# eps696/aphantasia

Measured on AMD Instinct MI355X. Metric: optimization steps/sec @1280x720 ViT-B/32 samples=200, higher is better.
Workload: dtype f16 (MFMA operands, fp32 accumulate; fp32 residual stream / LayerNorm / softmax statistics / synth / sampler / loss / Adam)

## Files before the change

aphantasia_amd/_ffi.py:

```python
import ctypes
import os
from ctypes import POINTER, c_char_p, c_float, c_int, c_size_t, c_void_p

import torch

HERE = os.path.dirname(os.path.abspath(__file__))
LIB_PATH = os.path.join(HERE, 'libaphantasia_hip.so')

APH_OUT_NCHW_RAW, APH_OUT_NCHW_NORM, APH_OUT_PATCH_F16, APH_GRAD_PATCH_F16, APH_OUT_PATCH_F16_HILO, APH_OUT_PATCH_F32 = 0, 1, 2, 3, 4, 5
APH_AUG_STRIDE = 16
SIM_TYPES = {'cossim': 0, 'cos': 0, None: 0, 'mix': 1, 'ang': 2, 'dot': 3}


class SampleGeom(ctypes.Structure):
    _fields_ = [(n, c_int) for n in ('H', 'W', 'Hp', 'Wp', 'py0', 'px0', 'S', 'size', 'patch')]


_PROTOTYPES = {
    'aph_version': (c_int, []),
    'aph_last_error': (c_char_p, []),
    'aph_synth_plan_create': (c_int, [c_int, c_int, c_int, POINTER(c_void_p)]),
    'aph_synth_plan_destroy': (c_int, [c_void_p]),
    'aph_synth_fft_fwd': (c_int, [c_void_p, c_void_p, c_void_p, c_void_p, c_float, POINTER(c_float), c_int, c_void_p, c_void_p, c_void_p]),
    'aph_synth_fft_bwd': (c_int, [c_void_p, c_void_p, c_float, c_void_p, c_void_p, c_void_p, c_float, POINTER(c_float), c_int, c_void_p, c_void_p]),
# ... 14 lines not shown
    'aph_idwt_level_bwd': (c_int, [c_void_p, c_int, c_int, c_int, c_void_p, c_void_p, c_int, c_float, c_void_p, c_int, c_int, c_void_p, c_void_p]),
    'aph_sample_ws_bytes': (c_size_t, [POINTER(SampleGeom), c_int]),
    'aph_sample_fwd': (c_int, [POINTER(SampleGeom), c_void_p, c_void_p, c_void_p, c_void_p, c_void_p, c_int, c_void_p]),
    'aph_sample_bwd': (c_int, [POINTER(SampleGeom), c_void_p, c_float, c_void_p, c_void_p, c_void_p, c_void_p, c_int, c_void_p]),
    'aph_triangle_blur': (c_int, [c_void_p, c_int, c_int, c_int, c_int, c_float, c_float, c_void_p, c_void_p]),
    'aph_resize_bicubic': (c_int, [c_void_p, c_int, c_int, c_int, c_void_p, c_int, c_int, c_void_p]),
    'aph_flip_w': (c_int, [c_void_p, c_void_p, c_int, c_int, c_int, c_void_p, c_void_p]),
    'aph_grid_warp': (c_int, [c_void_p, c_void_p, c_int, c_int, c_int, c_float, c_float, c_float, c_float, c_float, c_void_p, c_void_p, c_void_p]),
    'aph_attn_test': (c_int, [c_void_p, c_void_p, c_void_p, c_void_p, c_void_p, c_void_p, c_int, c_int, c_int, c_int, c_void_p]),
    'aph_attn_f32_test': (c_int, [c_void_p, c_void_p, c_void_p, c_void_p, c_void_p, c_void_p, c_int, c_int, c_int, c_int, c_void_p]),
    'aph_frame_affine': (c_int, [c_void_p, c_int, c_int, c_int, POINTER(c_float), c_void_p, c_void_p]),
    'aph_patchify_f16': (c_int, [c_void_p, c_int, c_int, c_int, c_void_p, c_void_p]),
    'aph_patchify_f16_hilo': (c_int, [c_void_p, c_int, c_int, c_int, c_void_p, c_void_p]),
    'aph_patchify_f32': (c_int, [c_void_p, c_int, c_int, c_int, c_void_p, c_void_p]),
    'aph_unpatchify_f32': (c_int, [c_void_p, c_int, c_int, c_int, c_float, c_void_p, c_void_p]),
    'aph_vit_create': (c_int, [c_int, c_int, c_int, c_int, c_int, c_int, c_int, POINTER(c_void_p)]),
    'aph_vit_destroy': (c_int, [c_void_p]),
    'aph_vit_workspace_bytes': (c_size_t, [c_void_p]),
    'aph_vit_set_weight': (c_int, [c_void_p, c_char_p, c_void_p, c_size_t]),
    'aph_vit_forward': (c_int, [c_void_p, c_void_p, c_int, c_void_p, c_void_p]),
    'aph_vit_forward_hilo': (c_int, [c_void_p, c_void_p, c_int, c_void_p, c_void_p]),
    'aph_vit_enable_hilo': (c_int, [c_void_p]),
    'aph_vit_enable_f32': (c_int, [c_void_p]),
    'aph_vit_forward_f32': (c_int, [c_void_p, c_void_p, c_int, c_void_p, c_void_p]),
    'aph_vit_backward_f32': (c_int, [c_void_p, c_void_p, c_int, c_void_p, c_float, c_void_p]),
    'aph_vit_backward': (c_int, [c_void_p, c_void_p, c_int, c_void_p, c_float, c_void_p]),
    'aph_vit_backward_h': (c_int, [c_void_p, c_void_p, c_int, c_void_p, c_float, c_void_p]),
    'aph_vit_profile': (c_int, [c_void_p, c_int]),
    'aph_vit_profile_read': (c_int, [c_void_p, c_void_p, c_void_p, c_void_p]),
    'aph_gemm_set_mfma32': (c_int, [c_int]),
    'aph_vit_set_fuse_ln': (c_int, [c_int]),
    'aph_crop_adjoint_set_gather': (c_int, [c_int]),
    'aph_crop_adjoint_set_shape': (c_int, [c_int, c_int, c_int, c_int, c_int]),
    'aph_vit_set_grad_stream_f16': (c_int, [c_int]),
    'aph_gemm_set_ws_min_tiles': (c_int, [c_int]),
    'aph_gemm_set_ws_pgroup': (c_int, [c_int]),
    'aph_gemm_set_rs': (c_int, [c_int]),
    'aph_mfma_rate': (c_int, [c_int, c_int, c_void_p, c_void_p, c_void_p]),
    'aph_gemm_rs_probe': (c_int, [c_void_p, c_void_p, c_int, c_int, c_int, c_void_p, c_int, c_void_p, c_void_p]),
    'aph_gemm_ws_probe': (c_int, [c_void_p, c_void_p, c_int, c_int, c_int, c_void_p, c_void_p, c_void_p, c_int, c_void_p, c_void_p]),
    'aph_gemm_f32_test': (c_int, [c_void_p, c_int, c_int, c_void_p, c_int, c_int, c_int, c_int, c_void_p, c_int, c_void_p, c_void_p, c_int, c_void_p, c_size_t, c_void_p]),
    'aph_gemm_f16': (c_int, [c_void_p, c_void_p, c_int, c_int, c_int, c_void_p, c_void_p]),
    'aph_gemm_f16_ld': (c_int, [c_void_p, c_int, c_void_p, c_int, c_int, c_int, c_int, c_void_p, c_int, c_void_p]),
    'aph_gemm_f16_epi_test': (c_int, [c_void_p, c_int, c_void_p, c_int, c_int, c_int, c_int, c_void_p, c_int, c_void_p, c_void_p, c_void_p, c_float, c_int,
                                      c_int, c_int, c_int, c_void_p, c_size_t, c_int, c_void_p]),
    'aph_ln_test': (c_int, [c_int, c_int, c_int, c_int, c_int, c_int, c_int, c_void_p, c_void_p, c_void_p, c_void_p, c_void_p, c_void_p, c_void_p,
                            c_void_p, c_void_p, c_void_p, c_void_p, c_void_p, c_void_p, c_void_p]),
    'aph_sim_loss': (c_int, [c_void_p, c_int, c_int, c_void_p, c_void_p, POINTER(c_float), c_int, c_int, c_int, c_int, c_int, c_float, c_float, c_void_p, c_void_p, c_void_p, c_void_p]),
    'aph_axpy_f32': (c_int, [c_void_p, c_void_p, c_float, c_size_t, c_void_p]),
    'aph_rgb_to_u8': (c_int, [c_void_p, c_int, c_int, c_float, c_void_p, c_void_p]),
    'aph_linear_head': (c_int, [c_void_p, c_int, c_int, c_void_p, c_float, c_float, c_float, c_float, c_void_p, c_void_p, c_void_p]),
    'aph_comm_unique_id': (c_int, [c_void_p]),
    'aph_comm_init': (c_int, [c_int, c_int, c_void_p, POINTER(c_void_p)]),
    'aph_allreduce_f32': (c_int, [c_void_p, c_void_p, c_size_t, c_void_p]),
    'aph_comm_ranks': (c_int, [c_void_p, POINTER(c_int)]),
    'aph_comm_destroy': (c_int, [c_void_p]),
    'aph_adam_step': (c_int, [c_void_p, c_void_p, c_void_p, c_void_p, c_void_p, c_void_p, c_int, c_size_t, c_void_p]),
    'aph_adam_step_guarded': (c_int, [c_void_p, c_void_p, c_void_p, c_void_p, c_void_p, c_void_p, c_int, c_size_t, c_void_p, c_void_p]),
}

EXPORTS = tuple(_PROTOTYPES)

class Library:

    def __init__(self, path):
        if not os.path.isfile(path):
# ... 45 lines not shown
```

aphantasia_amd/csrc/sampler.hip:

```cpp
#include <cstring>
#include <cstdlib>
#include <type_traits>

#include "sampler_layout.h"
#include "sampler_crop.h"
#include "sampler_crop_adjoint.h"
#include "sampler_warp.h"

namespace aph {

struct Nchw { int s, c, i, j; };
__device__ __forceinline__ Nchw nchw_of(size_t idx, int R) {
  return Nchw{(int)(idx / ((size_t)3 * R * R)), (int)((idx / ((size_t)R * R)) % 3), (int)((idx / R) % R), (int)(idx % R)};
}

__global__ void patchify_kernel(const float* __restrict__ x, half_t* __restrict__ out, int S, int R, int p, int hilo) {
  const size_t n = (size_t)S * 3 * R * R;
  const Layout<APH_OUT_PATCH_F16> L(R, p);
  for (size_t idx = (size_t)blockIdx.x * blockDim.x + threadIdx.x; idx < n; idx += (size_t)gridDim.x * blockDim.x) {
    const Nchw e = nchw_of(idx, R);
    const size_t o = L.index(e.s, e.c, e.i, e.j);
    const half_t h = (half_t)x[idx];
    if (!hilo) { out[o] = h; continue; }
    const size_t q = L.hilo_index(o);
// ... 20 lines not shown

using namespace aph;

static Geom to_geom(const aph_sample_geom* g) { return Geom{g->H, g->W, g->Hp, g->Wp, g->py0, g->px0, g->S, g->size, g->patch}; }

static int check_geom(const aph_sample_geom* g, int out_mode, const char* who, int max_mode = 2) {
  if (!g) return aph_fail(APH_ERR_ARG, "%s: null geometry", who);
  if (out_mode == APH_OUT_PATCH_F16_HILO && max_mode == 2) max_mode = APH_OUT_PATCH_F16_HILO;
  if (out_mode == APH_OUT_PATCH_F32) max_mode = APH_OUT_PATCH_F32;
  if (g->S < 1 || g->size < 1 || g->H < 1 || g->W < 1 || g->Hp < g->H || g->Wp < g->W)
    return aph_fail(APH_ERR_ARG, "%s: bad geometry S=%d size=%d H=%d W=%d Hp=%d Wp=%d", who, g->S, g->size, g->H, g->W, g->Hp, g->Wp);
  if (out_mode < 0 || out_mode > max_mode || (out_mode == APH_GRAD_PATCH_F16 && max_mode != APH_GRAD_PATCH_F16))
    return aph_fail(APH_ERR_ARG, "%s: bad out_mode %d", who, out_mode);
  if (out_mode >= APH_OUT_PATCH_F16 && (g->patch < 1 || g->size % g->patch || (g->patch & (g->patch - 1))))
    return aph_fail(APH_ERR_ARG, "%s: size %d not divisible by patch %d, or patch not a power of two", who, g->size, g->patch);
  return APH_OK;
}

namespace {
template <int... MODES> struct Modes {};
template <int... MODES, class F>
bool dispatch_out(Modes<MODES...>, int out_mode, F&& f) {
  return ((out_mode == MODES ? (f(std::integral_constant<int, MODES>{}), true) : false) || ...);
}
using FwdModes = Modes<APH_OUT_NCHW_RAW, APH_OUT_NCHW_NORM, APH_OUT_PATCH_F16, APH_OUT_PATCH_F32, APH_OUT_PATCH_F16_HILO>;
using GradModes = Modes<APH_OUT_NCHW_RAW, APH_OUT_NCHW_NORM, APH_OUT_PATCH_F16, APH_GRAD_PATCH_F16>;

size_t tab_bytes(const Geom& g) {
  const size_t maxcs = (size_t)(g.Hp < g.Wp ? g.Hp : g.Wp);
  return ((size_t)g.S * 2 * maxcs * sizeof(AdjEntry) + 255) & ~(size_t)255;
}
size_t scratch_floats(const Geom& g) { return (size_t)g.S * 4 * g.size * g.size; }
size_t strip_bytes(const Geom& g) { return ((size_t)(8 * (size_t)strip_cap(g) + 8) * sizeof(int) + 255) & ~(size_t)255; }
int* ws_strips(void* ws, const Geom& g) { return reinterpret_cast<int*>(static_cast<char*>(ws) + tab_bytes(g)); }
float* ws_scratch(void* ws, const Geom& g) { return reinterpret_cast<float*>(static_cast<char*>(ws) + tab_bytes(g) + strip_bytes(g)); }
}

extern "C" {

int aph_crop_adjoint_set_shape(int rb, int cpt, int nbc, int nseg, int order) {
  CropAdjointShape& v = crop_adjoint_shape();
  v.rb = rb; v.cpt = cpt; v.nbc = nbc; v.nseg = nseg; v.order = order;
  return APH_OK;
}
int aph_crop_adjoint_set_gather(int on) {
  const int prev = crop_adjoint_gather();
  crop_adjoint_gather() = on ? 1 : 0;
  return prev;
}

size_t aph_sample_ws_bytes(const aph_sample_geom* gg, int with_aug) {
  if (!gg || gg->S < 1 || gg->size < 1 || gg->Hp < 1 || gg->Wp < 1) return 0;
  const Geom g = to_geom(gg);
  return tab_bytes(g) + strip_bytes(g) + (with_aug ? 2 * scratch_floats(g) * sizeof(float) : 0);
}

int aph_sample_fwd(const aph_sample_geom* gg, const float* rgb, const int32_t* table_, const float* aug, void* ws,
                   void* out, int out_mode, void* stream_) {
  APH_TRY
  if (int e = check_geom(gg, out_mode, "aph_sample_fwd")) return e;
  if (!rgb || !table_ || !out || !ws) return aph_fail(APH_ERR_ARG, "aph_sample_fwd: null argument (the workspace of aph_sample_ws_bytes is required)");
  hipStream_t st = (hipStream_t)stream_;
  const Geom g = to_geom(gg);
  const int n = g.size;
  const int* table = (const int*)table_;
  int* strips = ws_strips(ws, g);
  if (!aug) {
    if (!dispatch_out(FwdModes{}, out_mode, [&](auto m) { launch_crop_resize<decltype(m)::value>(rgb, table, out, g, strips, st); })) return aph_fail(APH_ERR_ARG, "aph_sample_fwd: no kernel for out_mode %d", out_mode);
    return aph_check_launch("aph_sample_fwd");
  }
  float* A = ws_scratch(ws, g);
  float* Bv = A + scratch_floats(g);
  const dim3 grid((n + 31) / 32, (n + 7) / 8, g.S), block(256);
  launch_crop_resize<APH_SCRATCH_HWC4>(rgb, table, (void*)A, g, strips, st);
  APH_LAUNCH(persp_kernel, grid, block, 0, st, (const float*)A, aug, Bv, n);
  if (!dispatch_out(FwdModes{}, out_mode, [&](auto m) { APH_LAUNCH(rotate_emit_kernel<decltype(m)::value>, grid, block, 0, st, (const float*)A, (const float*)Bv, aug, out, n, g.patch); })) return aph_fail(APH_ERR_ARG, "aph_sample_fwd: no kernel for out_mode %d", out_mode);
  return aph_check_launch("aph_sample_fwd");
  APH_CATCH
}

int aph_sample_bwd(const aph_sample_geom* gg, const void* gout, float gscale, const int32_t* table_, const float* aug,
                   void* ws, float* grgb, int out_mode, void* stream_) {
  APH_TRY
  if (int e = check_geom(gg, out_mode, "aph_sample_bwd", APH_GRAD_PATCH_F16)) return e;
  if (out_mode == APH_OUT_PATCH_F32) out_mode = APH_OUT_PATCH_F16;
  if (!gout || !table_ || !grgb || !ws) return aph_fail(APH_ERR_ARG, "aph_sample_bwd: null argument (the workspace of aph_sample_ws_bytes is required)");
  hipStream_t st = (hipStream_t)stream_;
  const Geom g = to_geom(gg);
  const int n = g.size;
  const int* table = (const int*)table_;
  AdjEntry* tab = static_cast<AdjEntry*>(ws);
  int rc = APH_OK;
  if (!aug) {
    if (!dispatch_out(GradModes{}, out_mode, [&](auto m) { rc = launch_crop_adjoint<decltype(m)::value>(gout, gscale, table, grgb, g, tab, st); })) return aph_fail(APH_ERR_ARG, "aph_sample_bwd: no kernel for out_mode %d", out_mode);
    return rc ? rc : aph_check_launch("aph_sample_bwd");
  }
  float* dA = ws_scratch(ws, g);
  float* dB = dA + scratch_floats(g);
  const dim3 grid((n + 31) / 32, (n + 7) / 8, g.S), block(256);
  if (!dispatch_out(GradModes{}, out_mode, [&](auto m) { APH_LAUNCH(rotate_emit_adjoint_kernel<decltype(m)::value>, grid, block, 0, st, gout, aug, dA, dB, n, g.patch); })) return aph_fail(APH_ERR_ARG, "aph_sample_bwd: no kernel for out_mode %d", out_mode);
  APH_LAUNCH(persp_adjoint_kernel, grid, block, 0, st, (const float*)dB, aug, dA, n);
  rc = launch_crop_adjoint<APH_OUT_NCHW_RAW>((const void*)dA, gscale, table, grgb, g, tab, st);
  return rc ? rc : aph_check_launch("aph_sample_bwd");
  APH_CATCH
}

int aph_patchify_f16(const float* x, int S, int R, int patch, void* out, void* stream_) {
  APH_TRY
  if (!x || !out || S < 1 || R < 1 || patch < 1 || R % patch) return aph_fail(APH_ERR_ARG, "aph_patchify_f16: bad argument");
// ... 41 lines not shown
```

aphantasia_amd/csrc/sampler_crop.h:

```cpp
#pragma once
#include "sampler_layout.h"

namespace aph {

__device__ __forceinline__ void bicubic3(const float* __restrict__ rgb, const Geom& g, const CutBox& b, int i, int j, float v[3]) {
  const float sy = b.scale * (float)i, sx = b.scale * (float)j;
  const int y0 = (int)floorf(sy), x0 = (int)floorf(sx);
  float wy[4], wx[4];
  cubic_w(sy - (float)y0, wy);
  cubic_w(sx - (float)x0, wx);
  int ry[4], rx[4];
#pragma unroll
  for (int k = 0; k < 4; ++k) {
    int yy = y0 - 1 + k; yy = yy < 0 ? 0 : (yy > b.cs - 1 ? b.cs - 1 : yy);
    int xx = x0 - 1 + k; xx = xx < 0 ? 0 : (xx > b.cs - 1 ? b.cs - 1 : xx);
    ry[k] = wrap(b.oy + yy - g.py0, g.H);
    rx[k] = wrap(b.ox + xx - g.px0, g.W);
  }
  if (wave_all(rx[3] == rx[0] + 3)) {
    F4u t[3][4];
#pragma unroll
    for (int c = 0; c < 3; ++c)
#pragma unroll
      for (int a = 0; a < 4; ++a) t[c][a] = *reinterpret_cast<const F4u*>(rgb + ((size_t)c * g.H + ry[a]) * g.W + rx[0]);
#pragma unroll
    for (int c = 0; c < 3; ++c) {
      float acc = 0.f;
#pragma unroll
      for (int a = 0; a < 4; ++a) acc += (t[c][a].v[0] * wx[0] + t[c][a].v[1] * wx[1] + t[c][a].v[2] * wx[2] + t[c][a].v[3] * wx[3]) * wy[a];
      v[c] = acc;
    }
    return;
  }
#pragma unroll
// ... 2 lines not shown
    float acc = 0.f;
#pragma unroll
    for (int a = 0; a < 4; ++a) {
      const float* row = pl + (size_t)ry[a] * g.W;
      acc += (row[rx[0]] * wx[0] + row[rx[1]] * wx[1] + row[rx[2]] * wx[2] + row[rx[3]] * wx[3]) * wy[a];
    }
    v[c] = acc;
  }
}

constexpr int kStripPx = 16;
constexpr int kUnitRows = 4;
constexpr int kStripSlots = 768;

__global__ __launch_bounds__(1024) void strip_list_kernel(const int* __restrict__ table, int* __restrict__ lists, int* __restrict__ counts, int cap, Geom g, int strip_px) {
  __shared__ int cnt[8];
  if (threadIdx.x < 8) cnt[threadIdx.x] = 0;
  __syncthreads();
  const int groups = (g.size + kUnitRows - 1) / kUnitRows, units = g.S * groups;
  for (int u = threadIdx.x; u < units; u += blockDim.x) {
    const int s = u / groups, rg = u - s * groups;
    const CutBox b = load_cut(table, s, g.size);
    int i = rg * kUnitRows + kUnitRows / 2; i = i > g.size - 1 ? g.size - 1 : i;
    int yy = (int)floorf(b.scale * (float)i); yy = yy > b.cs - 1 ? b.cs - 1 : yy;
    const int yc = wrap(b.oy + yy - g.py0, g.H);
    const int xcd = (yc / strip_px) & 7;
    const int pos = atomicAdd(&cnt[xcd], 1);
    lists[xcd * cap + pos] = u;
  }
  __syncthreads();
  if (threadIdx.x < 8) counts[threadIdx.x] = cnt[threadIdx.x];
}

template <int OUT>
__global__ __launch_bounds__(256) void crop_resize_strips_kernel(const float* __restrict__ rgb, const int* __restrict__ table, void* __restrict__ out, Geom g,
                                                                 const int* __restrict__ lists, const int* __restrict__ counts, int cap) {
  const int xcd = blockIdx.x & 7, slot = blockIdx.x >> 3, nslot = gridDim.x >> 3;
  const int count = counts[xcd], groups = (g.size + kUnitRows - 1) / kUnitRows, n = g.size;
  for (int it = slot; it < count; it += nslot) {
    const int u = lists[xcd * cap + it];
    const int s = u / groups, rg = u - s * groups;
    const CutBox b = load_cut(table, s, n);
    for (int p = threadIdx.x; p < kUnitRows * n; p += blockDim.x) {
      const int di = p / n, j = p - di * n, i = rg * kUnitRows + di;
      if (i >= n) continue;
      float v[3];
      bicubic3(rgb, g, b, i, j, v);
      emit3<OUT>(out, s, i, j, n, g.patch, v[0], v[1], v[2]);
    }
  }
}

inline int strip_cap(const Geom& g) { return g.S * ((g.size + kUnitRows - 1) / kUnitRows); }

template <int OUT>
void launch_crop_resize(const float* rgb, const int* table, void* out, const Geom& g, int* lists, hipStream_t st) {
  int* counts = lists + 8 * (size_t)strip_cap(g);
  APH_LAUNCH(strip_list_kernel, dim3(1), dim3(1024), 0, st, table, lists, counts, strip_cap(g), g, kStripPx);
  APH_LAUNCH(crop_resize_strips_kernel<OUT>, dim3(8 * kStripSlots), dim3(256), 0, st, rgb, table, out, g, (const int*)lists, (const int*)counts, strip_cap(g));
}

}
```

aphantasia_amd/csrc/sampler_crop_adjoint.h:

```cpp
#pragma once
#include <type_traits>
#include "sampler_layout.h"

namespace aph {

struct AdjEntry { int off[4]; float w[4]; };

__device__ __forceinline__ float tap_weight(float scale, int i, int cs, int q) {
  const float sy = scale * (float)i;
  const int y0 = (int)floorf(sy);
  float wv[4];
  cubic_w(sy - (float)y0, wv);
  float w = 0.f;
#pragma unroll
  for (int k = 0; k < 4; ++k) {
    int yy = y0 - 1 + k; yy = yy < 0 ? 0 : (yy > cs - 1 ? cs - 1 : yy);
    if (yy == q) w += wv[k];
  }
  return w;
}

template <class Hit, class Put>
__device__ __forceinline__ void wave0_compact(int n, int* count, Hit hit, Put put) {
  int c = 0;
  for (int k0 = 0; k0 < n; k0 += 64) {
    const int k = k0 + (int)threadIdx.x;
    const bool h = k < n && hit(k);
    const unsigned long long m = __ballot(h);
    if (h) put(c + __popcll(m & ((1ull << threadIdx.x) - 1ull)), k);
    c += __popcll(m);
  }
  if (threadIdx.x == 0) *count = c;
}

template <int OUT, int NC>
__device__ __forceinline__ void upsample_cut_sum(const void* __restrict__ gout, size_t gb, const Layout<OUT>& L, float scale, int cs, int yc, int xc, float (&acc)[NC]) {
  for (int i = 0; i < L.size; ++i) {
    const float wy = tap_weight(scale, i, cs, yc);
    if (wy == 0.f) continue;
    for (int j = 0; j < L.size; ++j) {
      const float wx = tap_weight(scale, j, cs, xc);
      if (wx == 0.f) continue;
      const int o = L.rowpart(i) + L.colpart(j);
#pragma unroll
      for (int ch = 0; ch < NC; ++ch) acc[ch] += wy * wx * L.load(gout, gb + o + ch * L.chan_stride());
    }
  }
}

template <int OUT>
__global__ void tap_table_kernel(const int* __restrict__ table, AdjEntry* __restrict__ tab, int maxcs, Geom g) {
  const int s = blockIdx.z, isrow = blockIdx.y == 0;
  const int q = blockIdx.x * blockDim.x + threadIdx.x;
  const int cs = table[3 * s];
  if (q >= cs || q >= maxcs) return;
  const Layout<OUT> L(g.size, g.patch);
  AdjEntry e;
#pragma unroll
  for (int a = 0; a < 4; ++a) { e.off[a] = 0; e.w[a] = 0.f; }
  const float scale = cut_scale(cs, g.size);
  if (scale >= 1.0f) {
    const float inv = 1.0f / scale;
    int lo = (int)floorf((float)(q - 2) * inv) - 1, hi = (int)floorf((float)(q + 2) * inv) + 1;
    lo = lo < 0 ? 0 : lo; hi = hi > g.size - 1 ? g.size - 1 : hi;
    int n = 0;
    for (int i = lo; i <= hi && n < 4; ++i) {
      const float w = tap_weight(scale, i, cs, q);
      if (w != 0.f || n > 0) {
        e.w[n] = w;
        e.off[n] = isrow ? L.rowpart(i) : L.colpart(i);
        ++n;
      }
    }
  }
  tab[((size_t)s * 2 + (isrow ? 0 : 1)) * maxcs + q] = e;
}

template <int OUT>
__global__ __launch_bounds__(256) void crop_resize_adjoint_kernel(const void* __restrict__ gout, float gscale,
                                                                  const int* __restrict__ table, float* __restrict__ grgb, Geom g,
                                                                  const AdjEntry* __restrict__ tab, int maxcs) {
  constexpr int MAXV = 1024, NB = 8;
  __shared__ int vlist[MAXV];
  __shared__ int vcount;
  __shared__ AdjEntry ent[NB][32];
  __shared__ int vinfo[NB][3];
  const int tx = threadIdx.x & 15, ty = threadIdx.x >> 4;
  const int ntx_ = (g.W + 15) / 16, nty_ = (g.H + 15) / 16;
  const int xcd_ = blockIdx.x & 7, idx_ = blockIdx.x >> 3;
  const int lrow_ = idx_ / ntx_, bx_ = idx_ - lrow_ * ntx_, by_ = lrow_ * 8 + xcd_;
  if (by_ >= nty_) return;
  const int x = bx_ * 16 + tx, y = by_ * 16 + ty;
  const bool live = x < g.W && y < g.H;
  const int nay = (g.Hp + g.H - 1) / g.H, nax = (g.Wp + g.W - 1) / g.W;
  const int nvirt = g.S * nay * nax;
  const int ty0 = by_ * 16, tx0 = bx_ * 16;
  const Layout<OUT> L(g.size, g.patch);
  const int cchan = L.chan_stride(), ccut = L.cut_stride();
  float acc[3] = {0.f, 0.f, 0.f};
  for (int vbase = 0; vbase < nvirt; vbase += MAXV) {
    __syncthreads();
    if (threadIdx.x < 64) {
      wave0_compact(nvirt - vbase < MAXV ? nvirt - vbase : MAXV, &vcount, [&](int k) {
        const int v = vbase + k;
        const int s = v / (nay * nax), al = v - s * (nay * nax), ay = al / nax, ax = al - ay * nax;
        const int cs = table[3 * s], ox = table[3 * s + 1], oy = table[3 * s + 2];
        const int ylast = ty0 + 15 < g.H - 1 ? ty0 + 15 : g.H - 1, xlast = tx0 + 15 < g.W - 1 ? tx0 + 15 : g.W - 1;
        const int Ya = wrap(ty0 + g.py0, g.H) + ay * g.H, Yb = wrap(ylast + g.py0, g.H) + ay * g.H;
// ... 58 lines not shown
            if (ce.w[bq] == 0.f) continue;
            const float w = re.w[a] * ce.w[bq];
            const int o = re.off[a] + ce.off[bq];
            acc[0] += w * L.load(gout, gb + o);
            acc[1] += w * L.load(gout, gb + o + cchan);
            acc[2] += w * L.load(gout, gb + o + 2 * cchan);
          }
        }
      }
      __syncthreads();
    }
  }
  if (live) {
    const size_t HW = (size_t)g.H * g.W, o = (size_t)y * g.W + x;
    const float k0 = OUT == APH_OUT_NCHW_RAW ? gscale : gscale / kClipStd[0];
    const float k1 = OUT == APH_OUT_NCHW_RAW ? gscale : gscale / kClipStd[1];
    const float k2 = OUT == APH_OUT_NCHW_RAW ? gscale : gscale / kClipStd[2];
    grgb[o] = acc[0] * k0;
    grgb[HW + o] = acc[1] * k1;
    grgb[2 * HW + o] = acc[2] * k2;
  }
}

struct __attribute__((aligned(16))) QuadRow {
  float w[4];
  int off;
  int pad[3];
};
constexpr int ADJ_NBC = 12;

template <int OUT, int RBQ, int CPT>
__global__ __launch_bounds__(768) void crop_adjoint_rows_kernel(const void* __restrict__ gout, float gscale, const int* __restrict__ table,
                                                                 float* __restrict__ grgb, Geom g, const AdjEntry* __restrict__ tab, int maxcs,
                                                                 int RB, int NBC, int XW, int center_out) {
  constexpr int RBP = RBQ * 4, MAXV = 512;
  APH_DYN_SMEM(smem);
  float* U = reinterpret_cast<float*>(smem);
  QuadRow* qtab2 = reinterpret_cast<QuadRow*>(U + (size_t)NBC * g.size * RBP);
  int* binfo2 = reinterpret_cast<int*>(qtab2 + 2 * NBC * RBQ * 8);
  int* vlist = binfo2 + 2 * NBC * 4;
  int* vbox = vlist + MAXV;
  int* vcount = vbox + 3 * MAXV;
  const int tid = threadIdx.x, nthr = blockDim.x;
  const int nrb = gridDim.x, bi = blockIdx.x, rbi = center_out ? ((bi & 1) ? nrb / 2 - (bi + 1) / 2 : nrb / 2 + bi / 2) : bi;
  const int c = blockIdx.y, y0 = rbi * RB;
  const int x0 = blockIdx.z * XW, x1 = (x0 + XW < g.W ? x0 + XW : g.W);
  const int rows = g.H - y0 < RB ? g.H - y0 : RB;
  const Layout<OUT> L(g.size, g.patch);
  const int cchan = L.chan_stride(), ccut = L.cut_stride();
  f32x4 acc[CPT][RBQ];
#pragma unroll
  for (int i = 0; i < CPT; ++i)
#pragma unroll
    for (int k = 0; k < RBQ; ++k) acc[i][k] = f32x4{0.f, 0.f, 0.f, 0.f};
  for (int i = tid; i < NBC * g.size * RBP; i += nthr) U[i] = 0.f;
  for (int vbase = 0; vbase < g.S; vbase += MAXV) {
    __syncthreads();
    if (tid < 64) {
      int cs = 0, ox = 0, oy = 0;
      wave0_compact(g.S - vbase < MAXV ? g.S - vbase : MAXV, vcount, [&](int k) {
        const int s = vbase + k;
        cs = table[3 * s]; ox = table[3 * s + 1]; oy = table[3 * s + 2];
        return oy < y0 + rows && oy + cs > y0 && ox < x1 && ox + cs > x0;
      }, [&](int pos, int k) { vlist[pos] = vbase + k; vbox[3 * pos] = cs; vbox[3 * pos + 1] = ox; vbox[3 * pos + 2] = oy; });
    }
    __syncthreads();
    const int nlist = *vcount;
    constexpr int P0_THREADS = 256;
    const int p0_first = nthr - P0_THREADS;
    auto phase0 = [&](int b0, int buf) {
      if (tid < p0_first) return;
      QuadRow* qt = qtab2 + buf * NBC * RBQ * 8;
      int* bi = binfo2 + buf * NBC * 4;
      for (int pt = tid - p0_first; pt < NBC * RBQ * 8; pt += P0_THREADS) {
        const int b = pt / (RBQ * 8), qq = (pt >> 3) % RBQ, r = pt & 7;
        QuadRow qr;
        qr.off = -1; qr.w[0] = qr.w[1] = qr.w[2] = qr.w[3] = 0.f;
        if (b0 + b < nlist) {
          const int s = vlist[b0 + b];
          const int cs = vbox[3 * (b0 + b)], ox = vbox[3 * (b0 + b) + 1], oy = vbox[3 * (b0 + b) + 2];
          const bool generic = !(cut_scale(cs, g.size) >= 1.0f);
          if (qq == 0 && r == 0) { bi[4 * b] = s; bi[4 * b + 1] = generic ? -cs : cs; bi[4 * b + 2] = ox; bi[4 * b + 3] = oy; }
          if (!generic) {
            AdjEntry e[4];
            int i0[4], ilo = 1 << 30;
#pragma unroll
            for (int k = 0; k < 4; ++k) {
              const int q = 4 * qq + k, yc = y0 + q - oy;
              const bool live = q < rows && yc >= 0 && yc < cs && yc < maxcs;
              if (live) e[k] = tab[((size_t)s * 2) * maxcs + yc];
              i0[k] = 1 << 30;
              if (live && (e[k].w[0] != 0.f || e[k].w[1] != 0.f || e[k].w[2] != 0.f || e[k].w[3] != 0.f)) i0[k] = L.row_of(e[k].off[0]);
              else { e[k].w[0] = e[k].w[1] = e[k].w[2] = e[k].w[3] = 0.f; }
              ilo = i0[k] < ilo ? i0[k] : ilo;
            }
            if (ilo < (1 << 30)) {
              const int i = ilo + r;
              bool any = false;
#pragma unroll
              for (int k = 0; k < 4; ++k) {
                float w = 0.f;
#pragma unroll
                for (int a = 0; a < 4; ++a) w += (i0[k] + a == i) ? e[k].w[a] : 0.f;
                qr.w[k] = w;
                any = any || w != 0.f;
              }
              if (any && i < g.size) qr.off = L.rowpart(i);
            }
          }
        } else if (qq == 0 && r == 0) bi[4 * b] = -1;
        qt[pt] = qr;
      }
    };
    phase0(0, 0);
    __syncthreads();
    for (int b0 = 0, cur = 0; b0 < nlist; b0 += NBC, cur ^= 1) {
      const QuadRow* qtab = qtab2 + cur * NBC * RBQ * 8;
      const int* binfo = binfo2 + cur * NBC * 4;
      const int nb = nlist - b0 < NBC ? nlist - b0 : NBC;
      {
        const int lane = tid & 63, wv = tid >> 6, nwv = nthr >> 6, nquad = nb * RBQ;
        constexpr int JT = 4;
        unsigned colj[JT];
#pragma unroll
        for (int m = 0; m < JT; ++m) { const int j = lane + 64 * m; colj[m] = (unsigned)L.colpart(j < g.size ? j : 0); }
        for (int pq = wv; pq < nquad; pq += nwv) {
          float v[JT][8];
          const int b = pq / RBQ, qq = pq - b * RBQ;
          const size_t gb = (size_t)wave_uniform(binfo[4 * b]) * ccut + (size_t)c * cchan;
#pragma unroll
          for (int r = 0; r < 8; ++r) {
            const int off = wave_uniform(qtab[pq * 8 + r].off);
            const size_t rowbase = gb + (size_t)(off >= 0 ? off : 0);
#pragma unroll
            for (int m = 0; m < JT; ++m) {
              float x = 0.f;
              if (off >= 0 && lane + 64 * m < g.size) {
                if (OUT == APH_GRAD_PATCH_F16) x = (float)(reinterpret_cast<const half_t*>(gout) + rowbase)[colj[m]];
                else x = (reinterpret_cast<const float*>(gout) + rowbase)[colj[m]];
              }
              v[m][r] = x;
            }
          }
          f32x4 u[JT];
#pragma unroll
          for (int m = 0; m < JT; ++m) u[m] = f32x4{0.f, 0.f, 0.f, 0.f};
#pragma unroll
          for (int r = 0; r < 8; ++r) {
            const f32x4 w = *reinterpret_cast<const f32x4*>(qtab[pq * 8 + r].w);
#pragma unroll
            for (int m = 0; m < JT; ++m) u[m] += w * v[m][r];
          }
#pragma unroll
          for (int m = 0; m < JT; ++m) {
            const int j = lane + 64 * m;
            if (j < g.size) *reinterpret_cast<f32x4*>(U + ((size_t)b * g.size + j) * RBP + 4 * qq) = u[m];
          }
        }
      }
      __syncthreads();
      if (b0 + NBC < nlist) phase0(b0 + NBC, cur ^ 1);
      {
#pragma unroll
        for (int bh = 0; bh < ADJ_NBC; bh += 4) {
          if (bh >= nb) break;
          f32x4 cw[CPT][4];
          int coff[CPT][4];
#pragma unroll
          for (int i = 0; i < CPT; ++i) {
            const int x = x0 + i * nthr + tid;
#pragma unroll
            for (int bb = 0; bb < 4; ++bb) {
              const int b = bh + bb;
              coff[i][bb] = -1;
              cw[i][bb] = f32x4{0.f, 0.f, 0.f, 0.f};
              if (b < nb && x < x1) {
                const int s = binfo[4 * b], csx = binfo[4 * b + 1], p = x - binfo[4 * b + 2];
                if (csx > 0 && p >= 0 && p < csx && p < maxcs) {
                  const AdjEntry* ep = tab + ((size_t)s * 2 + 1) * maxcs + p;
                  coff[i][bb] = ep->off[0];
                  cw[i][bb] = *reinterpret_cast<const f32x4*>(ep->w);
                }
              }
            }
          }
#pragma unroll
          for (int i = 0; i < CPT; ++i)
#pragma unroll
            for (int bb = 0; bb < 4; ++bb) {
              if (coff[i][bb] < 0) continue;
              const float* u0 = U + ((size_t)(bh + bb) * g.size + L.col_of(coff[i][bb])) * RBP;
#pragma unroll
              for (int t = 0; t < 4; ++t) {
                if (cw[i][bb][t] == 0.f) continue;
                const float* up = u0 + t * RBP;
#pragma unroll
                for (int k = 0; k < RBQ; ++k) acc[i][k] += cw[i][bb][t] * *reinterpret_cast<const f32x4*>(up + 4 * k);
              }
            }
        }
#pragma unroll
        for (int i = 0; i < CPT; ++i) {
          const int x = x0 + i * nthr + tid;
          if (x >= x1) continue;
          for (int b = 0; b < nb; ++b) {
            const int csx = binfo[4 * b + 1];
            if (csx >= 0) continue;
            const int s = binfo[4 * b], oy = binfo[4 * b + 3], cs = -csx, p = x - binfo[4 * b + 2];
            if (p < 0 || p >= cs) continue;
            const float scale = cut_scale(cs, g.size);
            const size_t gb = (size_t)s * ccut + (size_t)c * cchan;
#pragma unroll
            for (int q = 0; q < RBP; ++q) {
              const int yc = y0 + q - oy;
              if (q >= rows || yc < 0 || yc >= cs) continue;
              float sum[1] = {0.f};
              upsample_cut_sum<OUT, 1>(gout, gb, L, scale, cs, yc, p, sum);
              acc[i][q >> 2][q & 3] += sum[0];
            }
          }
        }
      }
      __syncthreads();
    }
  }
  const float kc = OUT == APH_OUT_NCHW_RAW ? gscale : gscale / kClipStd[c];
  const size_t HW = (size_t)g.H * g.W;
#pragma unroll
  for (int i = 0; i < CPT; ++i) {
    const int x = x0 + i * nthr + tid;
    if (x >= x1) continue;
#pragma unroll
    for (int k = 0; k < RBQ; ++k)
#pragma unroll
      for (int r = 0; r < 4; ++r) {
        const int q = 4 * k + r;
        if (q < rows) grgb[(size_t)c * HW + (size_t)(y0 + q) * g.W + x] = acc[i][k][r] * kc;
      }
  }
}

inline int& crop_adjoint_gather() {
  static int v = 0;
  return v;
}

struct CropAdjointShape { int rb = 0, cpt = 0, nbc = 0, nseg = 0, order = -1; };
inline CropAdjointShape& crop_adjoint_shape() {
  static CropAdjointShape v;
  return v;
}
inline int device_cu_count() {
#ifdef APH_EMU
  return 3;
#else
  static const int n = [] { int dev = 0, cu = 256; if (hipGetDevice(&dev) == hipSuccess) (void)hipDeviceGetAttribute(&cu, hipDeviceAttributeMultiprocessorCount, dev); return cu > 0 ? cu : 256; }();
  return n;
#endif
}

template <int OUT>
int launch_crop_adjoint(const void* gout, float gscale, const int* table, float* grgb, const Geom& g, AdjEntry* tab, hipStream_t st) {
  const int maxcs = g.Hp < g.Wp ? g.Hp : g.Wp;
  APH_LAUNCH(tap_table_kernel<OUT>, dim3((maxcs + 127) / 128, 2, g.S), dim3(128), 0, st, table, tab, maxcs, g);
  if (!crop_adjoint_gather() && g.Hp == g.H && g.Wp == g.W && g.py0 == 0 && g.px0 == 0 && g.W <= 4 * 2304 && g.size <= 256) {
    int nseg = (g.W + 2303) / 2304;
    const CropAdjointShape& ov = crop_adjoint_shape();
    if (ov.nseg > 0) nseg = ov.nseg;
    const int xw = ((g.W + nseg - 1) / nseg + 3) & ~3;
    int cpt = xw <= 1536 ? 2 : 3;
    if (ov.cpt > 0) cpt = ov.cpt;
    int nthr = (((xw + cpt - 1) / cpt) + 63) / 64 * 64;
    nthr = nthr < 256 ? 256 : nthr;
    if (nthr > 768) return aph_fail(APH_ERR_ARG, "crop adjoint: %d columns per segment need more than 768 threads x %d columns", xw, cpt);
    int rb = (g.H + 84) / 85;
    rb = rb < 4 ? 4 : (rb > 16 ? 16 : rb);
    if (ov.rb > 0) rb = ov.rb;
    int rbq = rb <= 12 ? 3 : 4;
    const int rbp = rbq * 4;
    int nbc = ov.nbc > 0 && ov.nbc <= ADJ_NBC ? ov.nbc : ADJ_NBC;
    auto lds = [&](int n) { return (size_t)n * g.size * rbp * 4 + 2 * (size_t)n * rbq * 8 * sizeof(QuadRow) + 2 * (size_t)n * 16 + 512 * 16 + 16; };
    while (nbc > 1 && lds(nbc) > 150 * 1024) --nbc;
    if (lds(nbc) <= 150 * 1024) {
      const dim3 rgrid((g.H + rb - 1) / rb, 3, nseg);
      const size_t smem = lds(nbc);
      const int center_out = ov.order >= 0 ? ov.order : ((int)(rgrid.x * 3 * nseg) > device_cu_count() ? 1 : 0);
      auto rows = [&](auto rbq_, auto cpt_) {
        constexpr int RBQ = decltype(rbq_)::value, CPT = decltype(cpt_)::value;
        APH_ALLOW_SMEM((crop_adjoint_rows_kernel<OUT, RBQ, CPT>), 150 * 1024);
        APH_LAUNCH((crop_adjoint_rows_kernel<OUT, RBQ, CPT>), rgrid, dim3(nthr), smem, st, gout, gscale, table, grgb, g, (const AdjEntry*)tab, maxcs, rb, nbc, xw, center_out);
      };
      using I2 = std::integral_constant<int, 2>; using I3 = std::integral_constant<int, 3>; using I4 = std::integral_constant<int, 4>;
      if (rbq == 3 && cpt == 2) rows(I3{}, I2{});
      else if (rbq == 3) rows(I3{}, I3{});
      else if (cpt == 2) rows(I4{}, I2{});
      else rows(I4{}, I3{});
      return APH_OK;
    }
  }
  const dim3 agrid(8 * (((g.H + 15) / 16 + 7) / 8) * ((g.W + 15) / 16));
  APH_LAUNCH(crop_resize_adjoint_kernel<OUT>, agrid, dim3(256), 0, st, gout, gscale, table, grgb, g, (const AdjEntry*)tab, maxcs);
  return APH_OK;
}

}
```

aphantasia_amd/csrc/sampler_warp.h:

```cpp
#pragma once
#include "sampler_layout.h"

namespace aph {

struct Tap { int x0, y0; float wx0, wx1, wy0, wy1; };

__device__ __forceinline__ Tap make_tap(float gx, float gy, int w, int h) {
  const float ix = ((gx + 1.f) * (float)w - 1.f) * 0.5f;
  const float iy = ((gy + 1.f) * (float)h - 1.f) * 0.5f;
  Tap t;
  const float fx = floorf(ix), fy = floorf(iy);
  t.x0 = (int)fx; t.y0 = (int)fy;
  t.wx1 = ix - fx; t.wx0 = (fx + 1.f) - ix;
  t.wy1 = iy - fy; t.wy0 = (fy + 1.f) - iy;
  return t;
}
__device__ __forceinline__ Tap make_tap(float gx, float gy, int n) { return make_tap(gx, gy, n, n); }

__device__ __forceinline__ Tap persp_tap(const float* __restrict__ a, int i, int j, int n) {
  const float x = (float)j + 0.5f, y = (float)i + 0.5f, hn = 0.5f * (float)n;
  const float g1x = x * (a[0] / hn) + y * (a[1] / hn) + (a[2] / hn);
  const float g1y = x * (a[3] / hn) + y * (a[4] / hn) + (a[5] / hn);
  const float g2 = x * a[6] + y * a[7] + 1.0f;
  return make_tap(g1x / g2 - 1.0f, g1y / g2 - 1.0f, n);
// ... 17 lines not shown
__device__ __forceinline__ void warp_gather3(const float* __restrict__ src, const Tap& t, int n, const float* __restrict__ a, float v[3]) {
  float m = 0.f;
  v[0] = v[1] = v[2] = 0.f;
#pragma unroll
  for (int dy = 0; dy < 2; ++dy)
#pragma unroll
    for (int dx = 0; dx < 2; ++dx) {
      const int yy = t.y0 + dy, xx = t.x0 + dx;
      const bool in = yy >= 0 && yy < n && xx >= 0 && xx < n;
      const float w = in ? (dx ? t.wx1 : t.wx0) * (dy ? t.wy1 : t.wy0) : 0.f;
      const int yc = yy < 0 ? 0 : (yy > n - 1 ? n - 1 : yy), xc = xx < 0 ? 0 : (xx > n - 1 ? n - 1 : xx);
      const f32x4 sv = *reinterpret_cast<const f32x4*>(src + ((size_t)yc * n + xc) * 4);
      m += w;
      const float we = (ERASE && in_rect(a, yc, xc)) ? 0.f : w;
      v[0] += we * sv[0]; v[1] += we * sv[1]; v[2] += we * sv[2];
    }
  v[0] *= m; v[1] *= m; v[2] *= m;
}

__global__ void persp_kernel(const float* __restrict__ A, const float* __restrict__ aug, float* __restrict__ Bo, int n) {
  const int s = blockIdx.z;
  const float* a = aug + (size_t)s * APH_AUG_STRIDE;
  if (a[8] == 0.f) return;
  const int j = blockIdx.x * 32 + (threadIdx.x & 31), i = blockIdx.y * 8 + (threadIdx.x >> 5);
  if (i >= n || j >= n) return;
  const Tap t = persp_tap(a, i, j, n);
  float v[3];
  warp_gather3<false>(A + hwc4_index(s, 0, 0, n), t, n, a, v);
  *reinterpret_cast<f32x4*>(Bo + hwc4_index(s, i, j, n)) = f32x4{v[0], v[1], v[2], 0.f};
}

template <int OUT>
__global__ void rotate_emit_kernel(const float* __restrict__ A, const float* __restrict__ Bi, const float* __restrict__ aug,
                                   void* __restrict__ out, int n, int patch) {
  const int s = blockIdx.z;
  const float* a = aug + (size_t)s * APH_AUG_STRIDE;
  const int j = blockIdx.x * 32 + (threadIdx.x & 31), i = blockIdx.y * 8 + (threadIdx.x >> 5);
  if (i >= n || j >= n) return;
  const float* src = (a[8] != 0.f ? Bi : A) + hwc4_index(s, 0, 0, n);
  float v[3];
  if (a[15] != 0.f) {
    const Tap t = rot_tap(a[13], a[14], i, j, n);
    warp_gather3<true>(src, t, n, a, v);
  } else {
    const f32x4 q = *reinterpret_cast<const f32x4*>(src + ((size_t)i * n + j) * 4);
    const bool er = in_rect(a, i, j);
    v[0] = er ? 0.f : q[0]; v[1] = er ? 0.f : q[1]; v[2] = er ? 0.f : q[2];
  }
  emit3<OUT>(out, s, i, j, n, patch, v[0], v[1], v[2]);
}

__device__ __forceinline__ float tap_mask(const Tap& t, int n) {
  float m = 0.f;
  if (t.y0 >= 0 && t.y0 < n) { if (t.x0 >= 0 && t.x0 < n) m += t.wx0 * t.wy0; if (t.x0 + 1 >= 0 && t.x0 + 1 < n) m += t.wx1 * t.wy0; }
  if (t.y0 + 1 >= 0 && t.y0 + 1 < n) { if (t.x0 >= 0 && t.x0 < n) m += t.wx0 * t.wy1; if (t.x0 + 1 >= 0 && t.x0 + 1 < n) m += t.wx1 * t.wy1; }
  return m;
}
__device__ __forceinline__ float tap_hits(const Tap& t, int py, int px) {
  const int dy = py - t.y0, dx = px - t.x0;
  if (dy < 0 || dy > 1 || dx < 0 || dx > 1) return 0.f;
  return (dx ? t.wx1 : t.wx0) * (dy ? t.wy1 : t.wy0);
}

template <int OUT>
__global__ void rotate_emit_adjoint_kernel(const void* __restrict__ gout, const float* __restrict__ aug,
                                           float* __restrict__ dA, float* __restrict__ dB, int n, int patch) {
  const int s = blockIdx.z;
  const float* a = aug + (size_t)s * APH_AUG_STRIDE;
  const int px = blockIdx.x * 32 + (threadIdx.x & 31), py = blockIdx.y * 8 + (threadIdx.x >> 5);
// ... 144 lines not shown
```

Baseline: 159.1.

## Emit unaugmented samples directly from crop kernel and rebalance crop-adjoint row blocks

When a sample has neither perspective nor rotation augmentation, the crop/resize kernel now writes the final output with the erase mask applied, and the rotate/emit kernel skips that sample. This avoids the scratch round trip and the second pass for those samples. The crop adjoint now splits rows into variable 8- or 12-row quad blocks sized to the CU count so the grid fills the device in one wave. The tap table kernel also builds row and column entries in a single launch. The trade-off is extra template variants and added indexing complexity in the adjoint kernel.

```diff
diff --git a/aphantasia_amd/_ffi.py b/aphantasia_amd/_ffi.py
--- a/aphantasia_amd/_ffi.py
+++ b/aphantasia_amd/_ffi.py
@@ -70,6 +70,8 @@
     'aph_vit_set_fuse_ln': (c_int, [c_int]),
     'aph_crop_adjoint_set_gather': (c_int, [c_int]),
     'aph_crop_adjoint_set_shape': (c_int, [c_int, c_int, c_int, c_int, c_int]),
+    'aph_crop_adjoint_set_cus': (c_int, [c_int]),
+    'aph_sample_set_staged': (c_int, [c_int]),
     'aph_vit_set_grad_stream_f16': (c_int, [c_int]),
     'aph_gemm_set_ws_min_tiles': (c_int, [c_int]),
     'aph_gemm_set_ws_pgroup': (c_int, [c_int]),
diff --git a/aphantasia_amd/csrc/sampler.hip b/aphantasia_amd/csrc/sampler.hip
--- a/aphantasia_amd/csrc/sampler.hip
+++ b/aphantasia_amd/csrc/sampler.hip
@@ -76,6 +76,10 @@
 }
 size_t scratch_floats(const Geom& g) { return (size_t)g.S * 4 * g.size * g.size; }
 size_t strip_bytes(const Geom& g) { return ((size_t)(8 * (size_t)strip_cap(g) + 8) * sizeof(int) + 255) & ~(size_t)255; }
+int& sample_staged() {
+  static int v = 0;
+  return v;
+}
 int* ws_strips(void* ws, const Geom& g) { return reinterpret_cast<int*>(static_cast<char*>(ws) + tab_bytes(g)); }
 float* ws_scratch(void* ws, const Geom& g) { return reinterpret_cast<float*>(static_cast<char*>(ws) + tab_bytes(g) + strip_bytes(g)); }
 }
@@ -90,6 +94,17 @@
 int aph_crop_adjoint_set_gather(int on) {
   const int prev = crop_adjoint_gather();
   crop_adjoint_gather() = on ? 1 : 0;
+  return prev;
+}
+
+int aph_crop_adjoint_set_cus(int n) {
+  const int prev = crop_adjoint_cus();
+  crop_adjoint_cus() = n > 0 ? n : 0;
+  return prev;
+}
+int aph_sample_set_staged(int on) {
+  const int prev = sample_staged();
+  sample_staged() = on ? 1 : 0;
   return prev;
 }
 
@@ -116,9 +131,11 @@
   float* A = ws_scratch(ws, g);
   float* Bv = A + scratch_floats(g);
   const dim3 grid((n + 31) / 32, (n + 7) / 8, g.S), block(256);
-  launch_crop_resize<APH_SCRATCH_HWC4>(rgb, table, (void*)A, g, strips, st);
+  const int direct = sample_staged() ? 0 : 1;
+  if (!direct) launch_crop_resize<APH_SCRATCH_HWC4>(rgb, table, (void*)A, g, strips, st);
+  else if (!dispatch_out(FwdModes{}, out_mode, [&](auto m) { launch_crop_resize<APH_SCRATCH_HWC4, decltype(m)::value>(rgb, table, (void*)A, g, strips, st, aug, out); })) return aph_fail(APH_ERR_ARG, "aph_sample_fwd: no kernel for out_mode %d", out_mode);
   APH_LAUNCH(persp_kernel, grid, block, 0, st, (const float*)A, aug, Bv, n);
-  if (!dispatch_out(FwdModes{}, out_mode, [&](auto m) { APH_LAUNCH(rotate_emit_kernel<decltype(m)::value>, grid, block, 0, st, (const float*)A, (const float*)Bv, aug, out, n, g.patch); })) return aph_fail(APH_ERR_ARG, "aph_sample_fwd: no kernel for out_mode %d", out_mode);
+  if (!dispatch_out(FwdModes{}, out_mode, [&](auto m) { APH_LAUNCH(rotate_emit_kernel<decltype(m)::value>, grid, block, 0, st, (const float*)A, (const float*)Bv, aug, out, n, g.patch, direct); })) return aph_fail(APH_ERR_ARG, "aph_sample_fwd: no kernel for out_mode %d", out_mode);
   return aph_check_launch("aph_sample_fwd");
   APH_CATCH
 }
diff --git a/aphantasia_amd/csrc/sampler_crop.h b/aphantasia_amd/csrc/sampler_crop.h
--- a/aphantasia_amd/csrc/sampler_crop.h
+++ b/aphantasia_amd/csrc/sampler_crop.h
@@ -1,5 +1,6 @@
 #pragma once
 #include "sampler_layout.h"
+#include "sampler_warp.h"
 
 namespace aph {
 
@@ -68,32 +69,40 @@
   if (threadIdx.x < 8) counts[threadIdx.x] = cnt[threadIdx.x];
 }
 
-template <int OUT>
+template <int OUT, int DIRECT = -1>
 __global__ __launch_bounds__(256) void crop_resize_strips_kernel(const float* __restrict__ rgb, const int* __restrict__ table, void* __restrict__ out, Geom g,
-                                                                 const int* __restrict__ lists, const int* __restrict__ counts, int cap) {
+                                                                 const int* __restrict__ lists, const int* __restrict__ counts, int cap,
+                                                                 const float* __restrict__ aug = nullptr, void* __restrict__ direct_out = nullptr) {
   const int xcd = blockIdx.x & 7, slot = blockIdx.x >> 3, nslot = gridDim.x >> 3;
   const int count = counts[xcd], groups = (g.size + kUnitRows - 1) / kUnitRows, n = g.size;
   for (int it = slot; it < count; it += nslot) {
     const int u = lists[xcd * cap + it];
     const int s = u / groups, rg = u - s * groups;
     const CutBox b = load_cut(table, s, n);
+    const float* a = DIRECT >= 0 ? aug + (size_t)s * APH_AUG_STRIDE : nullptr;
+    const bool direct = DIRECT >= 0 && a[8] == 0.f && a[15] == 0.f;
     for (int p = threadIdx.x; p < kUnitRows * n; p += blockDim.x) {
       const int di = p / n, j = p - di * n, i = rg * kUnitRows + di;
       if (i >= n) continue;
       float v[3];
       bicubic3(rgb, g, b, i, j, v);
-      emit3<OUT>(out, s, i, j, n, g.patch, v[0], v[1], v[2]);
+      if (DIRECT >= 0 && direct) {
+        const bool er = in_rect(a, i, j);
+        emit3<(DIRECT >= 0 ? DIRECT : OUT)>(direct_out, s, i, j, n, g.patch, er ? 0.f : v[0], er ? 0.f : v[1], er ? 0.f : v[2]);
+      } else {
+        emit3<OUT>(out, s, i, j, n, g.patch, v[0], v[1], v[2]);
+      }
     }
   }
 }
 
 inline int strip_cap(const Geom& g) { return g.S * ((g.size + kUnitRows - 1) / kUnitRows); }
 
-template <int OUT>
-void launch_crop_resize(const float* rgb, const int* table, void* out, const Geom& g, int* lists, hipStream_t st) {
+template <int OUT, int DIRECT = -1>
+void launch_crop_resize(const float* rgb, const int* table, void* out, const Geom& g, int* lists, hipStream_t st, const float* aug = nullptr, void* direct_out = nullptr) {
   int* counts = lists + 8 * (size_t)strip_cap(g);
   APH_LAUNCH(strip_list_kernel, dim3(1), dim3(1024), 0, st, table, lists, counts, strip_cap(g), g, kStripPx);
-  APH_LAUNCH(crop_resize_strips_kernel<OUT>, dim3(8 * kStripSlots), dim3(256), 0, st, rgb, table, out, g, (const int*)lists, (const int*)counts, strip_cap(g));
+  APH_LAUNCH((crop_resize_strips_kernel<OUT, DIRECT>), dim3(8 * kStripSlots), dim3(256), 0, st, rgb, table, out, g, (const int*)lists, (const int*)counts, strip_cap(g), aug, direct_out);
 }
 
 }
diff --git a/aphantasia_amd/csrc/sampler_crop_adjoint.h b/aphantasia_amd/csrc/sampler_crop_adjoint.h
--- a/aphantasia_amd/csrc/sampler_crop_adjoint.h
+++ b/aphantasia_amd/csrc/sampler_crop_adjoint.h
@@ -50,7 +50,7 @@
 
 template <int OUT>
 __global__ void tap_table_kernel(const int* __restrict__ table, AdjEntry* __restrict__ tab, int maxcs, Geom g) {
-  const int s = blockIdx.z, isrow = blockIdx.y == 0;
+  const int s = blockIdx.z;
   const int q = blockIdx.x * blockDim.x + threadIdx.x;
   const int cs = table[3 * s];
   if (q >= cs || q >= maxcs) return;
@@ -59,21 +59,26 @@
 #pragma unroll
   for (int a = 0; a < 4; ++a) { e.off[a] = 0; e.w[a] = 0.f; }
   const float scale = cut_scale(cs, g.size);
+  int n = 0, i0 = 0;
   if (scale >= 1.0f) {
     const float inv = 1.0f / scale;
     int lo = (int)floorf((float)(q - 2) * inv) - 1, hi = (int)floorf((float)(q + 2) * inv) + 1;
     lo = lo < 0 ? 0 : lo; hi = hi > g.size - 1 ? g.size - 1 : hi;
-    int n = 0;
     for (int i = lo; i <= hi && n < 4; ++i) {
       const float w = tap_weight(scale, i, cs, q);
       if (w != 0.f || n > 0) {
+        if (n == 0) i0 = i;
         e.w[n] = w;
-        e.off[n] = isrow ? L.rowpart(i) : L.colpart(i);
         ++n;
       }
     }
   }
-  tab[((size_t)s * 2 + (isrow ? 0 : 1)) * maxcs + q] = e;
+  AdjEntry ec = e;
+#pragma unroll
+  for (int a = 0; a < 4; ++a)
+    if (a < n) { e.off[a] = L.rowpart(i0 + a); ec.off[a] = L.colpart(i0 + a); }
+  tab[((size_t)s * 2) * maxcs + q] = e;
+  tab[((size_t)s * 2 + 1) * maxcs + q] = ec;
 }
 
 template <int OUT>
@@ -198,7 +203,7 @@
 template <int OUT, int RBQ, int CPT>
 __global__ __launch_bounds__(768) void crop_adjoint_rows_kernel(const void* __restrict__ gout, float gscale, const int* __restrict__ table,
                                                                  float* __restrict__ grgb, Geom g, const AdjEntry* __restrict__ tab, int maxcs,
-                                                                 int RB, int NBC, int XW, int center_out) {
+                                                                 int RB, int NBC, int XW, int center_out, int top3, int nblk, int Q) {
   constexpr int RBP = RBQ * 4, MAXV = 512;
   APH_DYN_SMEM(smem);
   float* U = reinterpret_cast<float*>(smem);
@@ -209,9 +214,14 @@
   int* vcount = vbox + 3 * MAXV;
   const int tid = threadIdx.x, nthr = blockDim.x;
   const int nrb = gridDim.x, bi = blockIdx.x, rbi = center_out ? ((bi & 1) ? nrb / 2 - (bi + 1) / 2 : nrb / 2 + bi / 2) : bi;
-  const int c = blockIdx.y, y0 = rbi * RB;
+  const int bot3_first = nblk - (Q - 2 * nblk - top3);
+  const int quad0 = 2 * rbi + (rbi < top3 ? rbi : top3) + (rbi > bot3_first ? rbi - bot3_first : 0);
+  const int c = blockIdx.y, y0 = RB > 0 ? rbi * RB : 4 * quad0;
   const int x0 = blockIdx.z * XW, x1 = (x0 + XW < g.W ? x0 + XW : g.W);
-  const int rows = g.H - y0 < RB ? g.H - y0 : RB;
+  const int rbrows = RB > 0 ? RB : ((rbi < top3 || rbi >= bot3_first) ? 12 : 8);
+  const int rows = g.H - y0 < rbrows ? g.H - y0 : rbrows;
+  const int nq = (rows + 3) >> 2 < RBQ ? (rows + 3) >> 2 : RBQ;
+  auto div_nq = [&](int v) { return nq == 1 ? v : (nq == 2 ? v >> 1 : (nq == 3 ? v / 3 : v >> 2)); };
   const Layout<OUT> L(g.size, g.patch);
   const int cchan = L.chan_stride(), ccut = L.cut_stride();
   f32x4 acc[CPT][RBQ];
@@ -238,8 +248,8 @@
       if (tid < p0_first) return;
       QuadRow* qt = qtab2 + buf * NBC * RBQ * 8;
       int* bi = binfo2 + buf * NBC * 4;
-      for (int pt = tid - p0_first; pt < NBC * RBQ * 8; pt += P0_THREADS) {
-        const int b = pt / (RBQ * 8), qq = (pt >> 3) % RBQ, r = pt & 7;
+      for (int pt = tid - p0_first; pt < NBC * nq * 8; pt += P0_THREADS) {
+        const int b = div_nq(pt >> 3), qq = (pt >> 3) - b * nq, r = pt & 7;
         QuadRow qr;
         qr.off = -1; qr.w[0] = qr.w[1] = qr.w[2] = qr.w[3] = 0.f;
         if (b0 + b < nlist) {
@@ -285,14 +295,14 @@
       const int* binfo = binfo2 + cur * NBC * 4;
       const int nb = nlist - b0 < NBC ? nlist - b0 : NBC;
       {
-        const int lane = tid & 63, wv = tid >> 6, nwv = nthr >> 6, nquad = nb * RBQ;
+        const int lane = tid & 63, wv = tid >> 6, nwv = nthr >> 6, nquad = nb * nq;
         constexpr int JT = 4;
         unsigned colj[JT];
 #pragma unroll
         for (int m = 0; m < JT; ++m) { const int j = lane + 64 * m; colj[m] = (unsigned)L.colpart(j < g.size ? j : 0); }
         for (int pq = wv; pq < nquad; pq += nwv) {
           float v[JT][8];
-          const int b = pq / RBQ, qq = pq - b * RBQ;
+          const int b = div_nq(pq), qq = pq - b * nq;
           const size_t gb = (size_t)wave_uniform(binfo[4 * b]) * ccut + (size_t)c * cchan;
 #pragma unroll
           for (int r = 0; r < 8; ++r) {
@@ -327,6 +337,8 @@
       __syncthreads();
       if (b0 + NBC < nlist) phase0(b0 + NBC, cur ^ 1);
       {
+        auto row_taps = [&](auto nq_) {
+        constexpr int NQ = decltype(nq_)::value < RBQ ? decltype(nq_)::value : RBQ;
 #pragma unroll
         for (int bh = 0; bh < ADJ_NBC; bh += 4) {
           if (bh >= nb) break;
@@ -361,10 +373,13 @@
                 if (cw[i][bb][t] == 0.f) continue;
                 const float* up = u0 + t * RBP;
 #pragma unroll
-                for (int k = 0; k < RBQ; ++k) acc[i][k] += cw[i][bb][t] * *reinterpret_cast<const f32x4*>(up + 4 * k);
+                for (int k = 0; k < NQ; ++k) acc[i][k] += cw[i][bb][t] * *reinterpret_cast<const f32x4*>(up + 4 * k);
               }
             }
         }
+        };
+        if (CPT == 2 && nq <= 2) row_taps(std::integral_constant<int, CPT == 2 ? 2 : RBQ>{});
+        else row_taps(std::integral_constant<int, RBQ>{});
 #pragma unroll
         for (int i = 0; i < CPT; ++i) {
           const int x = x0 + i * nthr + tid;
@@ -397,12 +412,14 @@
     const int x = x0 + i * nthr + tid;
     if (x >= x1) continue;
 #pragma unroll
-    for (int k = 0; k < RBQ; ++k)
+    for (int k = 0; k < RBQ; ++k) {
+      if (k >= nq) continue;
 #pragma unroll
       for (int r = 0; r < 4; ++r) {
         const int q = 4 * k + r;
         if (q < rows) grgb[(size_t)c * HW + (size_t)(y0 + q) * g.W + x] = acc[i][k][r] * kc;
       }
+    }
   }
 }
 
@@ -424,11 +441,15 @@
   return n;
 #endif
 }
+inline int& crop_adjoint_cus() {
+  static int v = 0;
+  return v;
+}
 
 template <int OUT>
 int launch_crop_adjoint(const void* gout, float gscale, const int* table, float* grgb, const Geom& g, AdjEntry* tab, hipStream_t st) {
   const int maxcs = g.Hp < g.Wp ? g.Hp : g.Wp;
-  APH_LAUNCH(tap_table_kernel<OUT>, dim3((maxcs + 127) / 128, 2, g.S), dim3(128), 0, st, table, tab, maxcs, g);
+  APH_LAUNCH(tap_table_kernel<OUT>, dim3((maxcs + 127) / 128, 1, g.S), dim3(128), 0, st, table, tab, maxcs, g);
   if (!crop_adjoint_gather() && g.Hp == g.H && g.Wp == g.W && g.py0 == 0 && g.px0 == 0 && g.W <= 4 * 2304 && g.size <= 256) {
     int nseg = (g.W + 2303) / 2304;
     const CropAdjointShape& ov = crop_adjoint_shape();
@@ -443,18 +464,24 @@
     rb = rb < 4 ? 4 : (rb > 16 ? 16 : rb);
     if (ov.rb > 0) rb = ov.rb;
     int rbq = rb <= 12 ? 3 : 4;
+    const int cus = crop_adjoint_cus() > 0 ? crop_adjoint_cus() : device_cu_count();
+    const int Q = (g.H + 3) / 4;
+    const int nblk = cus / (3 * nseg) < Q / 2 ? cus / (3 * nseg) : Q / 2;
+    const bool quads = ov.rb <= 0 && nblk > 0 && Q <= 3 * nblk;
+    const int top3 = quads ? (Q - 2 * nblk) / 2 : 0;
+    if (quads) { rb = 0; rbq = 3; }
     const int rbp = rbq * 4;
     int nbc = ov.nbc > 0 && ov.nbc <= ADJ_NBC ? ov.nbc : ADJ_NBC;
     auto lds = [&](int n) { return (size_t)n * g.size * rbp * 4 + 2 * (size_t)n * rbq * 8 * sizeof(QuadRow) + 2 * (size_t)n * 16 + 512 * 16 + 16; };
     while (nbc > 1 && lds(nbc) > 150 * 1024) --nbc;
     if (lds(nbc) <= 150 * 1024) {
-      const dim3 rgrid((g.H + rb - 1) / rb, 3, nseg);
+      const dim3 rgrid(quads ? nblk : (g.H + rb - 1) / rb, 3, nseg);
       const size_t smem = lds(nbc);
-      const int center_out = ov.order >= 0 ? ov.order : ((int)(rgrid.x * 3 * nseg) > device_cu_count() ? 1 : 0);
+      const int center_out = ov.order >= 0 ? ov.order : ((int)(rgrid.x * 3 * nseg) > cus ? 1 : 0);
       auto rows = [&](auto rbq_, auto cpt_) {
         constexpr int RBQ = decltype(rbq_)::value, CPT = decltype(cpt_)::value;
         APH_ALLOW_SMEM((crop_adjoint_rows_kernel<OUT, RBQ, CPT>), 150 * 1024);
-        APH_LAUNCH((crop_adjoint_rows_kernel<OUT, RBQ, CPT>), rgrid, dim3(nthr), smem, st, gout, gscale, table, grgb, g, (const AdjEntry*)tab, maxcs, rb, nbc, xw, center_out);
+        APH_LAUNCH((crop_adjoint_rows_kernel<OUT, RBQ, CPT>), rgrid, dim3(nthr), smem, st, gout, gscale, table, grgb, g, (const AdjEntry*)tab, maxcs, rb, nbc, xw, center_out, top3, nblk, Q);
       };
       using I2 = std::integral_constant<int, 2>; using I3 = std::integral_constant<int, 3>; using I4 = std::integral_constant<int, 4>;
       if (rbq == 3 && cpt == 2) rows(I3{}, I2{});
diff --git a/aphantasia_amd/csrc/sampler_warp.h b/aphantasia_amd/csrc/sampler_warp.h
--- a/aphantasia_amd/csrc/sampler_warp.h
+++ b/aphantasia_amd/csrc/sampler_warp.h
@@ -73,9 +73,10 @@
 
 template <int OUT>
 __global__ void rotate_emit_kernel(const float* __restrict__ A, const float* __restrict__ Bi, const float* __restrict__ aug,
-                                   void* __restrict__ out, int n, int patch) {
-  const int s = blockIdx.z;
-  const float* a = aug + (size_t)s * APH_AUG_STRIDE;
+                                   void* __restrict__ out, int n, int patch, int direct) {
+  const int s = blockIdx.z;
+  const float* a = aug + (size_t)s * APH_AUG_STRIDE;
+  if (direct && a[8] == 0.f && a[15] == 0.f) return;
   const int j = blockIdx.x * 32 + (threadIdx.x & 31), i = blockIdx.y * 8 + (threadIdx.x >> 5);
   if (i >= n || j >= n) return;
   const float* src = (a[8] != 0.f ? Bi : A) + hwc4_index(s, 0, 0, n);
```

New measurement: 159.7 (median of 6 runs). No clear change (+0.4%).
